# xin-fight/Research-and-Implementation-of-Image-Dehazing-Algorithm-Based-on-Vision-Transformer

Hardware: AMD Instinct MI355X
Metric: train patches/sec (128x128, embed_dim=32) (higher is better)
Workload: dtype f32; 1 GPU; Uformer_ProbSparse train step E=32 ps=128 per-GPU bs=32 fp32 Charbonnier+CR(VGG19, seeded-random weights) + AdamW (BASELINE configs[1]); global_batch=32, parallelism=dp1, arithmetic=fp32 storage/accumulate; products 6xbf16 MFMA, dropped <= 2^-24, split_terms=6

## Files before the change

### include/dehaze_hip.h

```cpp
#ifndef DEHAZE_HIP_H
#define DEHAZE_HIP_H

#include <stdint.h>

#ifdef __cplusplus
extern "C" {
#endif

#define DHZ_OK 0
#define DHZ_EINVAL (-22)
#define DHZ_ELAUNCH (-5)

#define DHZ_F32 0
#define DHZ_BF16 1

#define DHZ_NTOK 64
#define DHZ_NTOP 25

int dhz_abi_version(void);
const char* dhz_last_error(void);
const char* dhz_build_id(void);
int dhz_set_reserved_cus(int k);
int dhz_get_reserved_cus(void);
int dhz_grid_cus(void);
// ... 161 lines not shown
int dhz_linear_wgrad(const float* dy, int ldy, const float* x, int ldx, int T, int N, int K,
                     float* dw, float* db, void* stream);
int dhz_linear_wgrad_rs(const float* dy, int ldy, const float* x, int ldx, int T, int N, int K, float* dw, float* db,
                        const float* row_scale, int rows_per_scale, void* stream);
int dhz_linear_wgrad_multi(const float* dy, int ldy, const float* x, int ldx, int T, int nmat, int nper, int K,
                           float* const* dw, float* const* db, void* stream);

int dhz_winograd_prepack(const float* weight, float* upack, int Kout, int Cin, int transposed_rot, void* stream);
int dhz_winograd_conv3x3(const float* x, const float* upack, const float* bias, int relu, const float* out_mask,
                         const float* out_addend, float* y, int B, int H, int W, int C, int K, void* stream);
int dhz_winograd43_prepack(const float* weight, float* upack, int Kout, int Cin, int transposed_rot, void* stream);
int dhz_winograd43_conv3x3(const float* x, const float* upack, const float* bias, int relu, const float* out_mask,
                           const float* out_addend, float* y, int B, int H, int W, int C, int K, void* stream);
int dhz_winograd43_conv3x3_pool(const float* x, const float* upack, const float* bias, float* ypool, float* scratch, int B, int H, int W,
                                int C, int K, void* stream);
int dhz_maxpool2x2_blocked_fwd(const float* x, float* y, int N, int H, int W, void* stream);
int dhz_maxpool2x2_blocked_bwd(const float* gy, const float* act, float* gx, int N, int H, int W, void* stream);
int dhz_layout_blocked8(const float* src, float* dst, int B, int C, int HW, int to_blocked, const float* bias, int relu,
                        void* stream);

int dhz_winograd_conv3x3_act(const float* x, const float* upack, const float* bias, int backward, const float* out_mask,
                             const float* out_addend, float* y, int B, int H, int W, int C, int K, void* stream);

int dhz_tokens_to_blocked8(const float* tok, int ld, const float* leaky_mask, float* blk, int B, int HW, int C, void* stream);
int dhz_blocked8_to_tokens(const float* blk, const float* addend, int ld_add, float* tok, int ld, int B, int HW, int C, void* stream);

size_t dhz_conv3x3_wgrad_workspace_bytes(int B, int H, int W, int Cin, int Kout);
int dhz_conv3x3_wgrad_parts(int B, int H, int W, int Cin, int Kout);
int dhz_conv3x3_wgrad(const float* x, const float* dy, float* dw, float* db, float* ws, size_t ws_bytes, int B, int H, int W, int Cin,
                      int Kout, void* stream);
// ... 120 lines not shown
```

### research-and-implementation-of-image-dehazing-algorithm-based-on-vision-transformer_amd/csrc/common.h

```cpp
#pragma once
#include <hip/hip_runtime.h>
#include <stdint.h>
#include <stdio.h>
#include "dehaze_hip.h"

typedef float f32x4 __attribute__((ext_vector_type(4)));
typedef float f32x16 __attribute__((ext_vector_type(16)));

struct bf16s { uint16_t v; };
__device__ __forceinline__ float bf16_to_f32(uint16_t h) { return __uint_as_float((uint32_t)h << 16); }
__device__ __forceinline__ uint16_t f32_to_bf16(float f) {
    const __bf16 b = (__bf16)f;
    return __builtin_bit_cast(uint16_t, b);
}
__device__ __forceinline__ float4 ld4(const float* p) { return *reinterpret_cast<const float4*>(p); }
#ifndef DHZ_ST4_NT
#define DHZ_ST4_NT 0
#endif
__device__ __forceinline__ void st4(float* p, float4 v) {
    if (DHZ_ST4_NT) __builtin_nontemporal_store(f32x4{v.x, v.y, v.z, v.w}, reinterpret_cast<f32x4*>(p));
    else *reinterpret_cast<float4*>(p) = v;
}
__device__ __forceinline__ float4 ld4(const bf16s* p) {
    const uint2 r = *reinterpret_cast<const uint2*>(p);
// ... 23 lines not shown
bool dhz_det();
int dhz_part_cus();
constexpr int DHZ_DET_MAXSEG = 8;
struct DetSegs {
    int n;
    long off[DHZ_DET_MAXSEG], len[DHZ_DET_MAXSEG];
    float* dst[DHZ_DET_MAXSEG];
};
float* dhz_det_ws(const char* who, long items, long slot);
int dhz_det_reduce(const char* who, const float* ws, int items, long slot, const DetSegs& segs, hipStream_t s);
template <bool DET>
__device__ __forceinline__ void dhz_accum(float* p, float v) {
    if constexpr (DET) *p = v;
    else atomicAdd(p, v);
}

#define DHZ_REQUIRE(cond, ...)            \
    do {                                  \
        if (!(cond)) {                    \
            dhz_set_error(__VA_ARGS__);   \
            return DHZ_EINVAL;            \
        }                                 \
    } while (0)

#define DHZ_CHECK_LAUNCH(name)                                                   \
    do {                                                                         \
        hipError_t e_ = hipGetLastError();                                       \
        if (e_ != hipSuccess) {                                                  \
            dhz_set_error("%s: launch failed: %s", name, hipGetErrorString(e_)); \
            return DHZ_ELAUNCH;                                                  \
// ... 119 lines not shown
```

### research-and-implementation-of-image-dehazing-algorithm-based-on-vision-transformer_amd/csrc/winograd43_conv.hip

```cpp
#include <stdlib.h>
#include <type_traits>
#include "common.h"

#ifndef W43_ABL
#define W43_ABL 0
#endif

namespace {

typedef float f32x2 __attribute__((ext_vector_type(2)));
typedef __attribute__((address_space(3))) void lds_void;
typedef const __attribute__((address_space(1))) void glb_void;

constexpr int KB = 32;
constexpr int CC = 8;
constexpr int NXI = 36;
constexpr int UF = NXI * CC * KB;
constexpr int NUBUF = 2;
constexpr int URUNS = UF / 256;
static_assert(URUNS / 4 == 9, "the counted wait at the end of a group (vmcnt(9)) leaves exactly a wave's filter requests in flight");
constexpr int PLANE = 332;
constexpr int PCHUNKS = 2 * PLANE;
constexpr int PRUNS = (PCHUNKS + 63) / 64;
constexpr int PFLOATS = PRUNS * 256;
// ... 42 lines not shown
__global__ __launch_bounds__(256, 1) void winograd43_conv3x3_kernel(const float* __restrict__ x, const float* __restrict__ upack,
                                                                    const float* __restrict__ bias, int relu,
                                                                    const float* __restrict__ out_mask,
                                                                    const float* __restrict__ out_addend, float* __restrict__ y, int H,
                                                                    int W, int C, int K, int nblk, int xcd_group, int cb0, int ncb,
                                                                    int chain, float* __restrict__ ypool) {
    extern __shared__ __attribute__((aligned(16))) float smem[];
    const int t = threadIdx.x, lane = t & 63;
    const int w = __builtin_amdgcn_readfirstlane(t >> 6);
    const int i16 = lane & 15, g = lane >> 4;
    const int ty = i16 >> 2, tx = i16 & 3, hf = g >> 1, sub = g & 1;
    float* const us = smem;
    float* const pw = smem + NUBUF * UF + w * PFLOATS;
    float* const bias_s = smem + NUBUF * UF + 4 * PFLOATS;
    const int KBn = K / KB, CBn = C / CC;
    int lid = blockIdx.x;
    if (xcd_group) lid = (blockIdx.x & 7) * (gridDim.x >> 3) + (blockIdx.x >> 3);
    const int kb = lid % KBn;
    int blk = (lid / KBn) * 4 + w;
    const bool live = blk < nblk;
    if (!live) blk = nblk - 1;
    const int bx_n = W / 16, by_n = H / 16;
    const int bimg = blk / (bx_n * by_n);
    const int by = (blk / bx_n) % by_n, bx = blk % bx_n;
    const int oy0 = by * 16, ox0 = bx * 16;
    const size_t plane = (size_t)H * W * 8;

    {
        f32x4* z = reinterpret_cast<f32x4*>(pw);
#pragma unroll
        for (int i = 0; i < PFLOATS / 4 / 64; ++i) z[lane + 64 * i] = f32x4{0.f, 0.f, 0.f, 0.f};
    }
    if (FWD && t < KB) bias_s[t] = bias ? bias[kb * KB + t] : 0.f;

    int poff[PRUNS];
#pragma unroll
    for (int r = 0; r < PRUNS; ++r) {
        const int c = 64 * r + lane;
        const int ph = c / PLANE, rr = c - ph * PLANE;
        const int k4 = rr / 73;
        const int q = rr - 73 * k4;
        const int row = 4 * k4 + q / 18, px = q % 18;
        const int iy = oy0 - 1 + row, ix = ox0 - 1 + px;
        const bool ok = ph < 2 && q < 72 && row < 18 && iy >= 0 && iy < H && ix >= 0 && ix < W;
        poff[r] = ok ? (iy * W + ix) * 8 + ph * 4 : -1;
    }
    const char* const xbase = reinterpret_cast<const char*>(x + ((size_t)bimg * CBn + cb0) * plane);
    const char* const ubase = reinterpret_cast<const char*>(upack + ((size_t)kb * CBn + cb0) * UF);
    const unsigned lane16 = lane * 16;
    auto dma_patch_run = [&](int cb, int r) {
        if (W43_ABL & 2) return;
        if (poff[r] >= 0) dma16s(xbase + (size_t)cb * plane * 4, (unsigned)(poff[r] * 4), pw + 256 * r);
    };
    auto dma_u_run = [&](int cb, int r) {
        if (W43_ABL & 2) return;
        const int run = w + 4 * r;
        dma16s(ubase + ((size_t)cb * UF + 256 * run) * 4, lane16, us + (cb & 1) * UF + 256 * run);
    };

    const float* const pread0 = pw + (hf * PLANE + 73 * ty + 4 * tx) * 4 + 2 * sub;
    constexpr int NXA = 32;
    f32x4 acc[NXA][2], accv[NXI - NXA][2];
// ... 236 lines not shown
        (void)hipFuncSetAttribute(reinterpret_cast<const void*>(&winograd43_conv3x3_kernel<F>),                        \
                                  hipFuncAttributeMaxDynamicSharedMemorySize, (int)W43_SMEM);                          \
        for (int cb0 = 0; cb0 < CBn; cb0 += CHAIN_GROUPS) {                                                            \
            const int ncb = CBn - cb0 < CHAIN_GROUPS ? CBn - cb0 : CHAIN_GROUPS;                                       \
            const int chain = (cb0 > 0 ? 1 : 0) | (cb0 + ncb < CBn ? 2 : 0);                                           \
            hipLaunchKernelGGL((winograd43_conv3x3_kernel<F>), dim3(grid), dim3(256), W43_SMEM, s, x, upack, bias,     \
                               relu, out_mask, out_addend, y, H, W, C, K, nblk, xcd_group, cb0, ncb, chain, ypool);    \
        }                                                                                                              \
    } while (0)
    if (fwd) GO(true); else GO(false);
#undef GO
    DHZ_CHECK_LAUNCH(who);
    return DHZ_OK;
}

extern "C" int dhz_winograd43_conv3x3(const float* x, const float* upack, const float* bias, int relu, const float* out_mask,
                                      const float* out_addend, float* y, int B, int H, int W, int C, int K, void* stream) {
    DHZ_REQUIRE(y, "dhz_winograd43_conv3x3: null pointer");
    return winograd43_launch("dhz_winograd43_conv3x3", x, upack, bias, relu, out_mask, out_addend, y, nullptr, B, H, W, C, K, stream);
}

extern "C" int dhz_winograd43_conv3x3_pool(const float* x, const float* upack, const float* bias, float* ypool, float* scratch, int B, int H,
                                           int W, int C, int K, void* stream) {
    DHZ_REQUIRE(ypool, "dhz_winograd43_conv3x3_pool: null pointer");
    return winograd43_launch("dhz_winograd43_conv3x3_pool", x, upack, bias, 1, nullptr, nullptr, scratch, ypool, B, H, W, C, K, stream);
}
```

### research-and-implementation-of-image-dehazing-algorithm-based-on-vision-transformer_amd/csrc/winograd_conv.hip

```cpp
#include <stdlib.h>
#include <type_traits>
#include "common.h"

#ifndef WINO_ABL
#define WINO_ABL 0
#endif

namespace {

typedef float f32x2 __attribute__((ext_vector_type(2)));

constexpr int KB = 32;
constexpr int CC = 8;
constexpr int RS = 48;
constexpr int PPL = 320;
constexpr int UF = 16 * CC * KB;
constexpr int VW = 16 * 4 * 32;
constexpr int WAVE_LDS = VW + 4 * PPL;
constexpr int YS = 68;
constexpr int NP4 = 4;
constexpr int NUBUF = 3;
constexpr size_t WINO_SMEM = (size_t)(NUBUF * UF + 8 * WAVE_LDS + KB) * sizeof(float);

__device__ __forceinline__ void wave_sync() {
    __builtin_amdgcn_fence(__ATOMIC_RELEASE, "wavefront");
    __builtin_amdgcn_wave_barrier();
    __builtin_amdgcn_fence(__ATOMIC_ACQUIRE, "wavefront");
}

constexpr float LEAKY_SLOPE = 0.01f;
template <bool FWD, bool Q8, bool LEAKY = false>
__global__ __launch_bounds__(512) void winograd_conv3x3_kernel(const float* __restrict__ x,
                                                           const float* __restrict__ upack,
                                                           const float* __restrict__ bias, int relu,
                                                           const float* __restrict__ out_mask,
                                                           const float* __restrict__ out_addend,
                                                           float* __restrict__ y, int H, int W, int C, int K, int nblk, int xcd_group,
                                                           int nimg) {
    extern __shared__ __attribute__((aligned(16))) float smem[];
    const int t = threadIdx.x, lane = t & 63, w = t >> 6, half = w >> 2, wl = w & 3;
    const int i16 = lane & 15, g = lane >> 4;
    float* us = smem;
    float* vw = smem + NUBUF * UF + w * WAVE_LDS;
    float* pw = vw + VW;
    const int KBn = K / KB, CBn = C / CC;
    int lid = blockIdx.x;
    if (xcd_group) lid = (blockIdx.x & 7) * (gridDim.x >> 3) + (blockIdx.x >> 3);
    const int kb = lid % KBn;
    int blk = (lid / KBn) * 2 + half;
    const bool live = blk < nblk;
    if (!live) blk = nblk - 1;
    const int bx_n = Q8 ? 1 : W / 16, by_n = Q8 ? 1 : H / 16;
    const int bimg = Q8 ? 0 : blk / (bx_n * by_n);
    const int by = (blk / bx_n) % by_n, bx = blk % bx_n;
    const int wy0 = by * 16 + 4 * wl, ox0 = bx * 16;
    const size_t plane = (size_t)H * W * 8;
    const int pbar = half ? 5 : 1;

    f32x4 acc[16][2];
#pragma unroll
    for (int xi = 0; xi < 16; ++xi) { acc[xi][0] = f32x4{0.f, 0.f, 0.f, 0.f}; acc[xi][1] = f32x4{0.f, 0.f, 0.f, 0.f}; }

// ... 9 lines not shown
        const bool in = e < 6 * 18 * 2 && iy >= 0 && iy < (Q8 ? 16 : H) && ix >= 0 && ix < (Q8 ? 16 : W);
        if (Q8) {
            const int img = min(4 * blk + 2 * (iy >> 3) + (ix >> 3), nimg - 1);
            poff[i] = in ? (unsigned)(img * (C / CC) * 512 + ((iy & 7) * 8 + (ix & 7)) * 8 + hf * 4) : 0u;
        } else
            poff[i] = in ? (unsigned)((iy * W + ix) * 8 + hf * 4) : 0u;
        pdst[i] = (2 * hf) * PPL + (in ? py * RS + px * 2 : 6 * RS + (lane & 15) * 2);
    }
    {
        float4* z = reinterpret_cast<float4*>(pw);
#pragma unroll
        for (int i = 0; i < 4 * PPL / 4 / 64; ++i) z[lane + 64 * i] = make_float4(0.f, 0.f, 0.f, 0.f);
    }
    float4 rp[NP4];
    float4 ru0, ru1;
    const float* xbase = x + (size_t)bimg * CBn * plane;
    const float4* ubase = reinterpret_cast<const float4*>(upack + (size_t)kb * CBn * UF) + t;
    auto gload_patch = [&](int cb) {
        const float* xp = xbase + (size_t)cb * plane;
#pragma unroll
        for (int i = 0; i < NP4; ++i) rp[i] = *reinterpret_cast<const float4*>(xp + poff[i]);
    };
    auto gload_u = [&](int cb) {
        const float4* up = ubase + (size_t)cb * (UF / 4);
        ru0 = up[0]; ru1 = up[512];
    };
    auto write_patch_slot = [&](int i) {
        const float4 val = rp[i];
        float* dst = pw + pdst[i];
        *reinterpret_cast<float2*>(dst) = make_float2(val.x, val.y);
        *reinterpret_cast<float2*>(dst + PPL) = make_float2(val.z, val.w);
    };
// ... 37 lines not shown
    };
    auto write_v = [&]() {
#pragma unroll
        for (int xi = 0; xi < 16; xi += 2) write_v2(xi);
    };

    float* bias_s = smem + NUBUF * UF + 8 * WAVE_LDS;
    if (FWD && t < KB) bias_s[t] = bias ? bias[kb * KB + t] : 0.f;

    gload_patch(0);
    gload_u(0);
    wave_sync();
#pragma unroll
    for (int i = 0; i < NP4; ++i) write_patch_slot(i);
    write_u(0);
    { const int c1 = CBn > 1 ? 1 : 0; gload_patch(c1); gload_u(c1); }
    wave_sync();
#pragma unroll
    for (int a = 0; a < 4; ++a) read_row(a);
#pragma unroll
    for (int b = 0; b < 4; ++b) col_transform(b);
#pragma unroll
    for (int a = 0; a < 4; ++a) row_transform(a);
    write_v();
    __syncthreads();

    const float* ufrag = us + (g * 16 + i16) * 4;
    const float* vfrag = vw + g * 32 + i16 * 2;
    auto group = [&](int cb, auto with_next) {
        constexpr bool WITH_NEXT = decltype(with_next)::value;
        const float* up = ufrag + (cb % NUBUF) * UF;
        const int nbuf = (cb + 1) % NUBUF;
        const int cb2 = cb + 2 < CBn ? cb + 2 : CBn - 1;
        auto slot = [&](int sidx) {
            if (!WITH_NEXT) return;
            if ((WINO_ABL & 1) && sidx >= 13 && sidx <= 21) return;
            if ((WINO_ABL & 2) && (sidx == 1 || sidx == 6)) { if (sidx == 6) wave_sync(); return; }
            if ((WINO_ABL & 8) && (sidx == 0 || (sidx >= 2 && sidx <= 5) || (sidx >= 8 && sidx <= 11) || sidx >= 22)) return;
            switch (sidx) {
                case 0: write_u(nbuf); break;
                case 1: gload_u(cb2); break;
                case 2: write_patch_slot(0); break;
                case 3: write_patch_slot(1); break;
                case 4: write_patch_slot(2); break;
                case 5: write_patch_slot(3); break;
                case 6: wave_sync(); gload_patch(cb2); break;
                case 8: read_row(0); break;
                case 9: read_row(1); break;
// ... 50 lines not shown
            __builtin_amdgcn_sched_barrier(0);
            slot(4 * j + 2);
            __builtin_amdgcn_sched_barrier(0);
            if (!(WINO_ABL & 4)) {
            acc[xi + 1][0] = mfma16(a1.y, b1.y, acc[xi + 1][0]);
            acc[xi + 1][1] = mfma16(a1.w, b1.y, acc[xi + 1][1]); } else { acc[xi + 1][1][0] += a1.y + b1.y + a1.z + a1.w; }
            __builtin_amdgcn_sched_barrier(0);
            slot(4 * j + 3);
            __builtin_amdgcn_sched_barrier(0);
            a0 = a0n; a1 = a1n; b0 = b0n; b1 = b1n;
        }
        wave_sync();
        if (WITH_NEXT && !(WINO_ABL & 8)) { write_v2(12); write_v2(14); }
        wave_sync();
    };
    for (int cb = 0; cb + 1 < CBn; ++cb) group(cb, std::true_type{});
    group(CBn - 1, std::false_type{});

    float* ys = vw;
    {
        const int ty = i16 >> 3, tx = i16 & 7;
        const float lo = relu ? 0.f : -__builtin_inff();
#pragma unroll
        for (int tr = 0; tr < 2; ++tr)
#pragma unroll
            for (int r = 0; r < 4; ++r) {
                const int k = 16 * tr + 4 * g + r;
                float m[16];
#pragma unroll
                for (int xi = 0; xi < 16; ++xi) m[xi] = acc[xi][tr][r];
                float t0[4], t1[4];
#pragma unroll
// ... 4 lines not shown
                const float bv = FWD ? bias_s[k] : 0.f;
                float y00 = t0[0] + t0[1] + t0[2] + bv, y01 = t0[1] - t0[2] - t0[3] + bv;
                float y10 = t1[0] + t1[1] + t1[2] + bv, y11 = t1[1] - t1[2] - t1[3] + bv;
                if (FWD && LEAKY) {
                    y00 = y00 > 0.f ? y00 : LEAKY_SLOPE * y00; y01 = y01 > 0.f ? y01 : LEAKY_SLOPE * y01;
                    y10 = y10 > 0.f ? y10 : LEAKY_SLOPE * y10; y11 = y11 > 0.f ? y11 : LEAKY_SLOPE * y11;
                } else if (FWD) { y00 = fmaxf(y00, lo); y01 = fmaxf(y01, lo); y10 = fmaxf(y10, lo); y11 = fmaxf(y11, lo); }
                float* o = ys + k * YS + (2 * ty) * 16 + 2 * tx;
                *reinterpret_cast<float2*>(o) = make_float2(y00, y01);
                *reinterpret_cast<float2*>(o + 16) = make_float2(y10, y11);
            }
    }
    wave_sync();
    if (live) {
        const int KG = K / 8;
#pragma unroll
        for (int i = 0; i < 8; ++i) {
            const int e = lane + 64 * i;
            const int hf = e & 1, px = (e >> 1) & 15, py = (e >> 5) & 3, kg = e >> 7;
            const float* s0 = ys + (kg * 8 + hf * 4) * YS + py * 16 + px;
            float4 v4 = make_float4(s0[0], s0[YS], s0[2 * YS], s0[3 * YS]);
            size_t o;
            if (Q8) {
                const int vy = wy0 + py, img = 4 * blk + 2 * (vy >> 3) + (px >> 3);
                if (img >= nimg) continue;
                o = ((((size_t)img * KG + kb * 4 + kg) * 8 + (vy & 7)) * 8 + (px & 7)) * 8 + hf * 4;
            } else
                o = (((size_t)bimg * KG + kb * 4 + kg) * H + wy0 + py) * W * 8 + (size_t)(ox0 + px) * 8 + hf * 4;
            if (!FWD || LEAKY) {
                if (out_addend) {
// ... 3 lines not shown
                if (LEAKY && !FWD && out_mask) {
                    const float4 m = *reinterpret_cast<const float4*>(out_mask + o);
                    v4.x = m.x > 0.f ? v4.x : LEAKY_SLOPE * v4.x; v4.y = m.y > 0.f ? v4.y : LEAKY_SLOPE * v4.y;
                    v4.z = m.z > 0.f ? v4.z : LEAKY_SLOPE * v4.z; v4.w = m.w > 0.f ? v4.w : LEAKY_SLOPE * v4.w;
                } else if (!FWD && out_mask) {
                    const float4 m = *reinterpret_cast<const float4*>(out_mask + o);
                    v4.x = m.x > 0.f ? v4.x : 0.f; v4.y = m.y > 0.f ? v4.y : 0.f;
                    v4.z = m.z > 0.f ? v4.z : 0.f; v4.w = m.w > 0.f ? v4.w : 0.f;
                }
            }
            *reinterpret_cast<float4*>(y + o) = v4;
        }
    }
}

__global__ void winograd_prepack_kernel(const float* __restrict__ wgt, float* __restrict__ upack, int Kout, int Cin,
                                        int transposed_rot) {
    const int e = blockIdx.x * blockDim.x + threadIdx.x;
    if (e >= Kout * Cin) return;
    const int k = e / Cin, c = e % Cin;
    float gk[3][3];
#pragma unroll
    for (int i = 0; i < 3; ++i)
#pragma unroll
        for (int j = 0; j < 3; ++j)
            gk[i][j] = transposed_rot ? wgt[((size_t)c * Kout + k) * 9 + (2 - i) * 3 + (2 - j)]
                                      : wgt[((size_t)k * Cin + c) * 9 + i * 3 + j];
    float tg[4][3];
#pragma unroll
    for (int j = 0; j < 3; ++j) {
// ... 121 lines not shown
    gx[o] = ra; gx[o + 2] = rb; gx[o + 2 * W] = rc; gx[o + 2 * W + 2] = rd;
}

}

extern "C" int dhz_winograd_prepack(const float* weight, float* upack, int Kout, int Cin, int transposed_rot,
                                    void* stream) {
    DHZ_REQUIRE(weight && upack && Kout % KB == 0 && Cin % CC == 0, "dhz_winograd_prepack: Kout=%d Cin=%d", Kout, Cin);
    const int n = Kout * Cin;
    hipLaunchKernelGGL(winograd_prepack_kernel, dim3((n + 255) / 256), dim3(256), 0, (hipStream_t)stream, weight, upack,
                       Kout, Cin, transposed_rot);
    DHZ_CHECK_LAUNCH("dhz_winograd_prepack");
    return DHZ_OK;
}

extern "C" int dhz_winograd_conv3x3(const float* x, const float* upack, const float* bias, int relu, const float* out_mask,
                                    const float* out_addend, float* y, int B, int H, int W, int C, int K, void* stream) {
    DHZ_REQUIRE(x && upack && y, "dhz_winograd_conv3x3: null pointer");
    const bool q8 = H == 8 && W == 8;
    DHZ_REQUIRE(B > 0 && ((H % 16 == 0 && W % 16 == 0) || q8) && C % CC == 0 && K % KB == 0,
                "dhz_winograd_conv3x3: unsupported shape B=%d H=%d W=%d C=%d K=%d", B, H, W, C, K);
    const bool fwd = !(out_mask || out_addend);
    DHZ_REQUIRE(fwd || !(bias || relu), "dhz_winograd_conv3x3: bias/relu and out_mask/out_addend are exclusive");
    const int nblk = q8 ? (B + 3) / 4 : B * (H / 16) * (W / 16);
    const int grid = ((nblk + 1) / 2) * (K / KB);
    hipStream_t s = (hipStream_t)stream;
#ifdef DHZ_DIAG
    static const int xcd_env = getenv("DHZ_WINO_XCD") ? atoi(getenv("DHZ_WINO_XCD")) : -1;
#else
    constexpr int xcd_env = -1;
#endif
    const int xcd_group = (grid % 8 == 0) && (xcd_env >= 0 ? xcd_env : 1);
#define GO(F, Q)                                                                                                   \
    do {                                                                                                           \
        (void)hipFuncSetAttribute(reinterpret_cast<const void*>(&winograd_conv3x3_kernel<F, Q>),                   \
                                  hipFuncAttributeMaxDynamicSharedMemorySize, (int)WINO_SMEM);                     \
        hipLaunchKernelGGL((winograd_conv3x3_kernel<F, Q>), dim3(grid), dim3(512), WINO_SMEM, s, x, upack, bias, relu, \
                           out_mask, out_addend, y, H, W, C, K, nblk, xcd_group, B);                               \
    } while (0)
    if (q8) { if (fwd) GO(true, true); else GO(false, true); }
    else { if (fwd) GO(true, false); else GO(false, false); }
#undef GO
    DHZ_CHECK_LAUNCH("dhz_winograd_conv3x3");
    return DHZ_OK;
}

extern "C" int dhz_winograd_conv3x3_act(const float* x, const float* upack, const float* bias, int backward, const float* out_mask,
                                        const float* out_addend, float* y, int B, int H, int W, int C, int K, void* stream) {
    DHZ_REQUIRE(x && upack && y, "dhz_winograd_conv3x3_act: null pointer");
    const bool q8 = H == 8 && W == 8;
    DHZ_REQUIRE(B > 0 && ((H % 16 == 0 && W % 16 == 0 && H > 0 && W > 0) || q8) && C > 0 && K > 0 && C % CC == 0 && K % KB == 0,
                "dhz_winograd_conv3x3_act: unsupported shape B=%d H=%d W=%d C=%d K=%d", B, H, W, C, K);
    DHZ_REQUIRE(backward ? (bias == nullptr && out_mask != nullptr) : out_mask == nullptr,
                "dhz_winograd_conv3x3_act: forward takes bias / out_addend, backward out_mask / out_addend");
    const int nblk = q8 ? (B + 3) / 4 : B * (H / 16) * (W / 16);
    const int grid = ((nblk + 1) / 2) * (K / KB);
    hipStream_t s = (hipStream_t)stream;
    const int xcd_group = grid % 8 == 0;
#define GO(F, Q)                                                                                                         \
    do {                                                                                                                 \
        (void)hipFuncSetAttribute(reinterpret_cast<const void*>(&winograd_conv3x3_kernel<F, Q, true>),                   \
                                  hipFuncAttributeMaxDynamicSharedMemorySize, (int)WINO_SMEM);                           \
        hipLaunchKernelGGL((winograd_conv3x3_kernel<F, Q, true>), dim3(grid), dim3(512), WINO_SMEM, s, x, upack, bias, 0, \
                           out_mask, out_addend, y, H, W, C, K, nblk, xcd_group, B);                                     \
    } while (0)
    if (q8) { if (!backward) GO(true, true); else GO(false, true); }
    else { if (!backward) GO(true, false); else GO(false, false); }
#undef GO
    DHZ_CHECK_LAUNCH("dhz_winograd_conv3x3_act");
    return DHZ_OK;
}

extern "C" int dhz_layout_blocked8(const float* src, float* dst, int B, int C, int HW, int to_blocked, const float* bias,
                                   int relu, void* stream) {
    DHZ_REQUIRE(src && dst && C % 8 == 0 && B > 0 && HW > 0, "dhz_layout_blocked8: bad arguments");
    DHZ_REQUIRE(to_blocked || !(bias || relu), "dhz_layout_blocked8: bias / relu only towards the blocked layout");
    const size_t n = (size_t)B * C * HW;
    if (HW % 4 == 0) {
        const size_t total = n / 32;
// ... 29 lines not shown
```

### research-and-implementation-of-image-dehazing-algorithm-based-on-vision-transformer_amd/dehaze_hip/_lib.py

```python
import ctypes
import os

_HERE = os.path.dirname(os.path.abspath(__file__))
LIB_PATH = os.environ.get("DHZ_LIB_PATH") or os.path.join(_HERE, "libdehaze_hip.so")

c_f = ctypes.c_void_p
c_p = ctypes.c_void_p
c_i = ctypes.c_int
c_l = ctypes.c_int64
c_fl = ctypes.c_float

SIGNATURES = {
    "dhz_abi_version": [],
    "dhz_last_error": [],
    "dhz_build_id": [],
    "dhz_set_reserved_cus": [ctypes.c_int],
    "dhz_gelu_fwd_dt": [ctypes.c_void_p, ctypes.c_void_p, ctypes.c_int64, ctypes.c_int, ctypes.c_void_p],
    "dhz_gelu_bwd_dt": [ctypes.c_void_p, ctypes.c_void_p, ctypes.c_void_p, ctypes.c_int64, ctypes.c_void_p, ctypes.c_int64, ctypes.c_int, ctypes.c_void_p],
    "dhz_get_reserved_cus": [],
    "dhz_set_deterministic": [ctypes.c_int],
    "dhz_get_deterministic": [],
    "dhz_set_det_workspace": [ctypes.c_void_p, ctypes.c_size_t],
    "dhz_grid_cus": [],
    "dhz_ps_attn_fwd": [c_f, c_f, c_f, c_i, c_p, c_f, c_f, c_f, c_i, c_p, c_i, c_i, c_i, c_i, c_p],
# ... 21 lines not shown
    "dhz_thin_conv3x3_fwd": [c_f, c_f, c_f, c_f, c_i, c_i, c_i, c_i, c_p],
    "dhz_thin_conv3x3_dgrad": [c_f, c_f, c_f, c_i, c_i, c_i, c_i, c_p],
    "dhz_conv3x3_in3_blocked": [c_f, c_f, c_f, c_f, c_i, c_i, c_i, c_i, c_i, c_p],
    "dhz_thin_conv3x3_dgrad_blocked": [c_f, c_f, c_f, c_i, c_i, c_i, c_i, c_p],
    "dhz_thin_conv3x3_wgrad": [c_f, c_f, c_f, c_f, c_i, c_i, c_i, c_i, c_p],
    "dhz_l1_pair_fwd": [c_f, c_f, c_f, c_f, c_l, c_p],
    "dhz_l1_pair_bwd": [c_f, c_f, c_f, c_f, c_f, c_l, c_p],
    "dhz_contrast_combine_fwd": [c_f, c_f, c_f, c_i, c_i, c_f, c_f, c_p],
    "dhz_contrast_combine_bwd": [c_f, c_f, c_i, c_i, c_f, c_f, c_f, c_f, c_p],
    "dhz_crop_augment_pair": [c_f, c_f, c_f, c_f, c_f, c_i, c_i, c_i, c_i, c_p],
    "dhz_winograd_prepack": [c_f, c_f, c_i, c_i, c_i, c_p],
    "dhz_winograd_conv3x3": [c_f, c_f, c_f, c_i, c_f, c_f, c_f, c_i, c_i, c_i, c_i, c_i, c_p],
    "dhz_winograd43_prepack": [c_f, c_f, c_i, c_i, c_i, c_p],
    "dhz_winograd43_conv3x3": [c_f, c_f, c_f, c_i, c_f, c_f, c_f, c_i, c_i, c_i, c_i, c_i, c_p],
    "dhz_winograd43_conv3x3_pool": [c_f, c_f, c_f, c_f, c_f, c_i, c_i, c_i, c_i, c_i, c_p],
    "dhz_maxpool2x2_blocked_fwd": [c_f, c_f, c_i, c_i, c_i, c_p],
    "dhz_maxpool2x2_blocked_bwd": [c_f, c_f, c_f, c_i, c_i, c_i, c_p],
    "dhz_layout_blocked8": [c_f, c_f, c_i, c_i, c_i, c_i, c_f, c_i, c_p],
    "dhz_leff_fused_fwd": [c_f] * 16 + [c_i, c_i, c_i, c_i, c_p],
    "dhz_leff_fused_fwd6": [c_f] * 15 + [c_i, c_i, c_i, c_i, c_p],
    "dhz_leff_prepack6": [c_f, c_f, c_p, c_i, c_p],
    "dhz_linear_fwd": [c_f, c_i, c_f, c_f, c_f, c_i, c_i, c_i, c_i, c_p],
    "dhz_linear_dgrad": [c_f, c_i, c_f, c_f, c_i, c_i, c_i, c_i, c_p],
    "dhz_input_proj_fwd": [c_f, c_f, c_f, c_f, c_i, c_i, c_i, c_i, c_fl, c_p],
    "dhz_input_proj_bwd": [c_f, c_f, c_f, c_f, c_f, c_i, c_i, c_i, c_i, c_fl, c_p],
    "dhz_conv4s2_fwd": [c_f, c_f, c_f, c_f, c_i, c_i, c_i, c_i, c_i, c_p],
    "dhz_conv4s2_dgrad": [c_f, c_f, c_f, c_i, c_i, c_i, c_i, c_i, c_p],
    "dhz_conv4s2_wgrad": [c_f, c_f, c_f, c_f, c_i, c_i, c_i, c_i, c_i, c_p],
    "dhz_input_proj_fwd_dt": [c_f, c_f, c_f, c_f, c_i, c_i, c_i, c_i, c_fl, c_i, c_p],
    "dhz_input_proj_bwd_dt": [c_f, c_f, c_f, c_f, c_f, c_i, c_i, c_i, c_i, c_fl, c_i, c_p],
# ... 127 lines not shown
```

### research-and-implementation-of-image-dehazing-algorithm-based-on-vision-transformer_amd/dehaze_hip/vgg.py

```python
import os

import torch
import torch.nn.functional as F
from torch.autograd import Function

from . import _lib
from . import ops
from .ops import _p, _stream

CONVS = ((3, 64), (64, 64), (64, 128), (128, 128), (128, 256), (256, 256), (256, 256), (256, 256), (256, 512),
         (512, 512), (512, 512), (512, 512), (512, 512))
POOL_AFTER = (1, 3, 7, 11)
TAPS = (0, 2, 4, 8, 12)


def wino_supported(H, W):
    return (H % 16 == 0 and W % 16 == 0) or (H == 8 and W == 8)


def to_blocked(x, bias=None, relu=False):
    B, C, H, W = x.shape
    out = torch.empty((B, C // 8, H, W, 8), device=x.device, dtype=torch.float32)
    _lib.call("dhz_layout_blocked8", _p(x.contiguous()), _p(out), B, C, H * W, 1, _p(bias), int(relu), _stream())
    return out
# ... 27 lines not shown

F43_ON = os.environ.get("DHZ_WINO_F43", "1") != "0"


F43_DIFF = os.environ.get("DHZ_WINO_F43_DIFF", "1") != "0"
POOL_FUSED = os.environ.get("DHZ_WINO_POOL", "1") != "0"


def use_f43(B, H, W, Cin, Kout):
    if not F43_ON or H % 16 or W % 16 or H < 16 or W < 16 or Cin % 16 or Kout % 32:
        return False
    wgs = (B * (H // 16) * (W // 16) + 3) // 4 * (Kout // 32)
    cus = _lib.load().dhz_grid_cus() + _lib.load().dhz_get_reserved_cus()
    rounds = (wgs + cus - 1) // cus
    return wgs >= 0.92 * rounds * cus


class VggEngine:
    def __init__(self, convs):
        self.convs = convs
        self._packed = {}
        self._packed43 = {}

    def packed(self, i, device):
        key = (i, str(device), self.convs[i].weight.data_ptr(), self.convs[i].weight._version)
        hit = self._packed.get(i)
        if hit is None or hit[0] != key:
            w = self.convs[i].weight.detach().contiguous()
            K, C = w.shape[0], w.shape[1]
            uf = torch.empty(16 * K * C, device=device, dtype=torch.float32)
# ... 10 lines not shown
        if hit is None or hit[0] != key:
            w = self.convs[i].weight.detach().contiguous()
            K, C = w.shape[0], w.shape[1]
            uf = torch.empty(36 * K * C, device=device, dtype=torch.float32)
            ub = torch.empty(36 * K * C, device=device, dtype=torch.float32)
            _lib.call("dhz_winograd43_prepack", _p(w), _p(uf), K, C, 0, _stream())
            _lib.call("dhz_winograd43_prepack", _p(w), _p(ub), C, K, 1, _stream())
            hit = (key, uf, ub)
            self._packed43[i] = hit
        return hit[1], hit[2]

    def conv(self, i, xb, allow43=True, pool=False):
        B, CG, H, W, _ = xb.shape
        C, K = CONVS[i]
        f43 = allow43 and use_f43(B, H, W, C, K)
        uf, _ = self.packed43(i, xb.device) if f43 else self.packed(i, xb.device)
        if pool and f43:
            yp = torch.empty((B, K // 8, H // 2, W // 2, 8), device=xb.device, dtype=torch.float32)
            scratch = torch.empty((B, K // 8, H, W, 8), device=xb.device, dtype=torch.float32) if C > 256 else None
            ev = ops._timed("dhz_winograd_conv3x3")
            _lib.call("dhz_winograd43_conv3x3_pool", _p(xb), _p(uf), _p(self.convs[i].bias), _p(yp), _p(scratch) if scratch is not None else None,
                      B, H, W, C, K, _stream())
            _timing_end(ev, B, H, W, C, K, f43)
            return yp
        yb = torch.empty((B, K // 8, H, W, 8), device=xb.device, dtype=torch.float32)
        ev = ops._timed("dhz_winograd_conv3x3")
        _lib.call("dhz_winograd43_conv3x3" if f43 else "dhz_winograd_conv3x3", _p(xb), _p(uf), _p(self.convs[i].bias), 1, None, None,
                  _p(yb), B, H, W, C, K, _stream())
        _timing_end(ev, B, H, W, C, K, f43)
        return pool_fwd(yb) if pool else yb

    def conv_dgrad(self, i, gb, below_act=None, addend=None):
        B, KG, H, W, _ = gb.shape
        C, K = CONVS[i]
        f43 = use_f43(B, H, W, K, C)
        _, ub = self.packed43(i, gb.device) if f43 else self.packed(i, gb.device)
        dxb = torch.empty((B, C // 8, H, W, 8), device=gb.device, dtype=torch.float32)
        ev = ops._timed("dhz_winograd_conv3x3")
        _lib.call("dhz_winograd43_conv3x3" if f43 else "dhz_winograd_conv3x3", _p(gb), _p(ub), None, 0,
                  _p(below_act) if below_act is not None else None,
                  _p(addend.contiguous()) if addend is not None else None, _p(dxb), B, H, W, K, C, _stream())
        _timing_end(ev, B, H, W, K, C, f43)
        return dxb

    def forward_taps(self, x, save=None):
        c0 = self.convs[0]
        xc = x.contiguous()
        cur = torch.empty((xc.shape[0], 8, xc.shape[2], xc.shape[3], 8), device=x.device, dtype=torch.float32)
        _lib.call("dhz_conv3x3_in3_blocked", _p(xc), _p(c0.weight.contiguous()), _p(c0.bias), _p(cur), xc.shape[0], xc.shape[2],
                  xc.shape[3], 64, 1, _stream())
        acts = {0: cur}
        taps = [cur]
        x12 = None
        for i in range(1, 13):
            if i == 12 and not wino_supported(cur.shape[2], cur.shape[3]):
                c12 = self.convs[12]
                ops.warn_library_fallback("VGG19 conv5_1", tuple(cur.shape))
# ... 302 lines not shown
```

Baseline: 1004 patches/s.

## Split Winograd VGG convs over input-channel slices with a reduction epilogue

Adds split-K style slicing of the Winograd F(2,3) and F(4,3) conv kernels over input-channel groups. Each slice writes raw partial sums to a workspace, and a separate epilogue kernel sums them and applies bias/ReLU or mask/addend. Slicing is chosen only when the normal grid underfills the CUs, so deep low-resolution VGG layers get more workgroups. The cost is extra workspace traffic, one more kernel launch per conv, and a different summation order.

```diff
diff --git a/include/dehaze_hip.h b/include/dehaze_hip.h
--- a/include/dehaze_hip.h
+++ b/include/dehaze_hip.h
@@ -199,6 +199,13 @@
                            const float* out_addend, float* y, int B, int H, int W, int C, int K, void* stream);
 int dhz_winograd43_conv3x3_pool(const float* x, const float* upack, const float* bias, float* ypool, float* scratch, int B, int H, int W,
                                 int C, int K, void* stream);
+int dhz_winograd_conv3x3_slices(const float* x, const float* upack, const float* bias, int relu, const float* out_mask,
+                                const float* out_addend, float* y, float* workspace, int slices, int B, int H, int W, int C, int K,
+                                void* stream);
+int dhz_winograd43_conv3x3_slices(const float* x, const float* upack, const float* bias, int relu, const float* out_mask,
+                                  const float* out_addend, float* y, float* workspace, int slices, int B, int H, int W, int C, int K,
+                                  void* stream);
+int dhz_winograd_slices(int B, int H, int W, int C, int K);
 int dhz_maxpool2x2_blocked_fwd(const float* x, float* y, int N, int H, int W, void* stream);
 int dhz_maxpool2x2_blocked_bwd(const float* gy, const float* act, float* gx, int N, int H, int W, void* stream);
 int dhz_layout_blocked8(const float* src, float* dst, int B, int C, int HW, int to_blocked, const float* bias, int relu,
diff --git a/research-and-implementation-of-image-dehazing-algorithm-based-on-vision-transformer_amd/csrc/common.h b/research-and-implementation-of-image-dehazing-algorithm-based-on-vision-transformer_amd/csrc/common.h
--- a/research-and-implementation-of-image-dehazing-algorithm-based-on-vision-transformer_amd/csrc/common.h
+++ b/research-and-implementation-of-image-dehazing-algorithm-based-on-vision-transformer_amd/csrc/common.h
@@ -61,6 +61,9 @@
     if constexpr (DET) *p = v;
     else atomicAdd(p, v);
 }
+
+int dhz_wino_slices_epilogue(const char* who, const float* ws, int slices, const float* bias, int relu, const float* out_mask,
+                             const float* out_addend, float* y, int B, int H, int W, int K, hipStream_t s);
 
 #define DHZ_REQUIRE(cond, ...)            \
     do {                                  \
diff --git a/research-and-implementation-of-image-dehazing-algorithm-based-on-vision-transformer_amd/csrc/winograd43_conv.hip b/research-and-implementation-of-image-dehazing-algorithm-based-on-vision-transformer_amd/csrc/winograd43_conv.hip
--- a/research-and-implementation-of-image-dehazing-algorithm-based-on-vision-transformer_amd/csrc/winograd43_conv.hip
+++ b/research-and-implementation-of-image-dehazing-algorithm-based-on-vision-transformer_amd/csrc/winograd43_conv.hip
@@ -80,6 +80,8 @@
     float* const pw = smem + NUBUF * UF + w * PFLOATS;
     float* const bias_s = smem + NUBUF * UF + 4 * PFLOATS;
     const int KBn = K / KB, CBn = C / CC;
+    const int sl = blockIdx.y;
+    cb0 += sl * ncb;
     int lid = blockIdx.x;
     if (xcd_group) lid = (blockIdx.x & 7) * (gridDim.x >> 3) + (blockIdx.x >> 3);
     const int kb = lid % KBn;
@@ -87,7 +89,8 @@
     const bool live = blk < nblk;
     if (!live) blk = nblk - 1;
     const int bx_n = W / 16, by_n = H / 16;
-    const int bimg = blk / (bx_n * by_n);
+    const int bimg_in = blk / (bx_n * by_n);
+    const int bimg = bimg_in + sl * (nblk / (bx_n * by_n));
     const int by = (blk / bx_n) % by_n, bx = blk % bx_n;
     const int oy0 = by * 16, ox0 = bx * 16;
     const size_t plane = (size_t)H * W * 8;
@@ -111,7 +114,7 @@
         const bool ok = ph < 2 && q < 72 && row < 18 && iy >= 0 && iy < H && ix >= 0 && ix < W;
         poff[r] = ok ? (iy * W + ix) * 8 + ph * 4 : -1;
     }
-    const char* const xbase = reinterpret_cast<const char*>(x + ((size_t)bimg * CBn + cb0) * plane);
+    const char* const xbase = reinterpret_cast<const char*>(x + ((size_t)bimg_in * CBn + cb0) * plane);
     const char* const ubase = reinterpret_cast<const char*>(upack + ((size_t)kb * CBn + cb0) * UF);
     const unsigned lane16 = lane * 16;
     auto dma_patch_run = [&](int cb, int r) {
@@ -378,6 +381,31 @@
     return DHZ_OK;
 }
 
+extern "C" int dhz_winograd43_conv3x3_slices(const float* x, const float* upack, const float* bias, int relu, const float* out_mask,
+                                             const float* out_addend, float* y, float* workspace, int slices, int B, int H, int W, int C,
+                                             int K, void* stream) {
+    const char* who = "dhz_winograd43_conv3x3_slices";
+    DHZ_REQUIRE(x && upack && y && workspace, "%s: null pointer", who);
+    DHZ_REQUIRE(B > 0 && H % 16 == 0 && W % 16 == 0 && H >= 16 && W >= 16 && C > 0 && K > 0 && C % 16 == 0 && K % KB == 0,
+                "%s: unsupported shape B=%d H=%d W=%d C=%d K=%d", who, B, H, W, C, K);
+    const bool fwd = !(out_mask || out_addend);
+    DHZ_REQUIRE(fwd || !(bias || relu), "%s: bias/relu and out_mask/out_addend are exclusive", who);
+    DHZ_REQUIRE((long long)H * W * 8 * (C / 8) < (1ll << 31), "%s: image too large", who);
+    const int CBn = C / CC;
+    DHZ_REQUIRE(slices >= 2 && slices <= 64 && CBn % slices == 0 && CBn / slices <= CHAIN_GROUPS,
+                "%s: slices=%d of %d channel groups (equal ranges of at most %d)", who, slices, CBn, CHAIN_GROUPS);
+    const long long nblk = (long long)B * (H / 16) * (W / 16);
+    const long long grid1 = ((nblk + 3) / 4) * (K / KB);
+    DHZ_REQUIRE(grid1 * slices < (1ll << 31) && nblk * slices < (1ll << 31) / 4, "%s: grid too large", who);
+    const int xcd_group = (grid1 % 8 == 0) ? 1 : 0;
+    (void)hipFuncSetAttribute(reinterpret_cast<const void*>(&winograd43_conv3x3_kernel<false>), hipFuncAttributeMaxDynamicSharedMemorySize,
+                              (int)W43_SMEM);
+    hipLaunchKernelGGL((winograd43_conv3x3_kernel<false>), dim3((unsigned)grid1, (unsigned)slices), dim3(256), W43_SMEM, (hipStream_t)stream,
+                       x, upack, nullptr, 0, nullptr, nullptr, workspace, H, W, C, K, (int)nblk, xcd_group, 0, CBn / slices, 2, nullptr);
+    DHZ_CHECK_LAUNCH(who);
+    return dhz_wino_slices_epilogue(who, workspace, slices, bias, relu, out_mask, out_addend, y, B, H, W, K, (hipStream_t)stream);
+}
+
 extern "C" int dhz_winograd43_conv3x3(const float* x, const float* upack, const float* bias, int relu, const float* out_mask,
                                       const float* out_addend, float* y, int B, int H, int W, int C, int K, void* stream) {
     DHZ_REQUIRE(y, "dhz_winograd43_conv3x3: null pointer");
diff --git a/research-and-implementation-of-image-dehazing-algorithm-based-on-vision-transformer_amd/csrc/winograd_conv.hip b/research-and-implementation-of-image-dehazing-algorithm-based-on-vision-transformer_amd/csrc/winograd_conv.hip
--- a/research-and-implementation-of-image-dehazing-algorithm-based-on-vision-transformer_amd/csrc/winograd_conv.hip
+++ b/research-and-implementation-of-image-dehazing-algorithm-based-on-vision-transformer_amd/csrc/winograd_conv.hip
@@ -29,14 +29,14 @@
 }
 
 constexpr float LEAKY_SLOPE = 0.01f;
-template <bool FWD, bool Q8, bool LEAKY = false>
+template <bool FWD, bool Q8, bool LEAKY = false, bool RAW = false>
 __global__ __launch_bounds__(512) void winograd_conv3x3_kernel(const float* __restrict__ x,
                                                            const float* __restrict__ upack,
                                                            const float* __restrict__ bias, int relu,
                                                            const float* __restrict__ out_mask,
                                                            const float* __restrict__ out_addend,
                                                            float* __restrict__ y, int H, int W, int C, int K, int nblk, int xcd_group,
-                                                           int nimg) {
+                                                           int nimg, int slices) {
     extern __shared__ __attribute__((aligned(16))) float smem[];
     const int t = threadIdx.x, lane = t & 63, w = t >> 6, half = w >> 2, wl = w & 3;
     const int i16 = lane & 15, g = lane >> 4;
@@ -44,8 +44,13 @@
     float* vw = smem + NUBUF * UF + w * WAVE_LDS;
     float* pw = vw + VW;
     const int KBn = K / KB, CBn = C / CC;
-    int lid = blockIdx.x;
-    if (xcd_group) lid = (blockIdx.x & 7) * (gridDim.x >> 3) + (blockIdx.x >> 3);
+    static_assert(!RAW || (!FWD && !LEAKY), "the raw store is the backward instance without mask and addend");
+    const int grid1 = RAW ? (int)gridDim.x / slices : (int)gridDim.x;
+    const int sl = RAW ? (int)blockIdx.x / grid1 : 0;
+    int lid = RAW ? (int)blockIdx.x - sl * grid1 : (int)blockIdx.x;
+    if (xcd_group) lid = (lid & 7) * (grid1 >> 3) + (lid >> 3);
+    const int cbs = RAW ? sl * CBn / slices : 0;
+    const int NG = RAW ? (sl + 1) * CBn / slices - cbs : CBn;
     const int kb = lid % KBn;
     int blk = (lid / KBn) * 2 + half;
     const bool live = blk < nblk;
@@ -85,8 +90,8 @@
     }
     float4 rp[NP4];
     float4 ru0, ru1;
-    const float* xbase = x + (size_t)bimg * CBn * plane;
-    const float4* ubase = reinterpret_cast<const float4*>(upack + (size_t)kb * CBn * UF) + t;
+    const float* xbase = x + ((size_t)bimg * CBn + cbs) * plane;
+    const float4* ubase = reinterpret_cast<const float4*>(upack + ((size_t)kb * CBn + cbs) * UF) + t;
     auto gload_patch = [&](int cb) {
         const float* xp = xbase + (size_t)cb * plane;
 #pragma unroll
@@ -154,7 +159,7 @@
 #pragma unroll
     for (int i = 0; i < NP4; ++i) write_patch_slot(i);
     write_u(0);
-    { const int c1 = CBn > 1 ? 1 : 0; gload_patch(c1); gload_u(c1); }
+    { const int c1 = NG > 1 ? 1 : 0; gload_patch(c1); gload_u(c1); }
     wave_sync();
 #pragma unroll
     for (int a = 0; a < 4; ++a) read_row(a);
@@ -171,7 +176,7 @@
         constexpr bool WITH_NEXT = decltype(with_next)::value;
         const float* up = ufrag + (cb % NUBUF) * UF;
         const int nbuf = (cb + 1) % NUBUF;
-        const int cb2 = cb + 2 < CBn ? cb + 2 : CBn - 1;
+        const int cb2 = cb + 2 < NG ? cb + 2 : NG - 1;
         auto slot = [&](int sidx) {
             if (!WITH_NEXT) return;
             if ((WINO_ABL & 1) && sidx >= 13 && sidx <= 21) return;
@@ -252,8 +257,8 @@
         if (WITH_NEXT && !(WINO_ABL & 8)) { write_v2(12); write_v2(14); }
         wave_sync();
     };
-    for (int cb = 0; cb + 1 < CBn; ++cb) group(cb, std::true_type{});
-    group(CBn - 1, std::false_type{});
+    for (int cb = 0; cb + 1 < NG; ++cb) group(cb, std::true_type{});
+    group(NG - 1, std::false_type{});
 
     float* ys = vw;
     {
@@ -288,6 +293,7 @@
     wave_sync();
     if (live) {
         const int KG = K / 8;
+        if (RAW) y += (size_t)sl * nimg * K * H * W;
 #pragma unroll
         for (int i = 0; i < 8; ++i) {
             const int e = lane + 64 * i;
@@ -321,6 +327,40 @@
     }
 }
 
+template <bool FWD>
+__global__ __launch_bounds__(256) void winograd_slices_epilogue_kernel(const float4* __restrict__ ws, size_t n4, int slices,
+                                                                       const float* __restrict__ bias, int relu,
+                                                                       const float4* __restrict__ out_mask,
+                                                                       const float4* __restrict__ out_addend, float4* __restrict__ y,
+                                                                       int HW, int KG) {
+    const size_t e = (size_t)blockIdx.x * 256 + threadIdx.x;
+    if (e >= n4) return;
+    float4 r = make_float4(0.f, 0.f, 0.f, 0.f);
+    if (slices > 1) r = ws[e];
+    for (int s = 1; s + 1 < slices; ++s) {
+        const float4 p = ws[(size_t)s * n4 + e];
+        r.x += p.x; r.y += p.y; r.z += p.z; r.w += p.w;
+    }
+    float4 v = ws[(size_t)(slices - 1) * n4 + e];
+    if (FWD) {
+        float4 b = make_float4(0.f, 0.f, 0.f, 0.f);
+        if (bias) b = *reinterpret_cast<const float4*>(bias + ((e >> 1) / HW % KG) * 8 + (e & 1) * 4);
+        v.x += b.x; v.y += b.y; v.z += b.z; v.w += b.w;
+    }
+    if (slices > 1) { v.x += r.x; v.y += r.y; v.z += r.z; v.w += r.w; }
+    if (FWD) {
+        const float lo = relu ? 0.f : -__builtin_inff();
+        v.x = fmaxf(v.x, lo); v.y = fmaxf(v.y, lo); v.z = fmaxf(v.z, lo); v.w = fmaxf(v.w, lo);
+    } else {
+        if (out_addend) { const float4 ad = out_addend[e]; v.x += ad.x; v.y += ad.y; v.z += ad.z; v.w += ad.w; }
+        if (out_mask) {
+            const float4 m = out_mask[e];
+            v.x = m.x > 0.f ? v.x : 0.f; v.y = m.y > 0.f ? v.y : 0.f; v.z = m.z > 0.f ? v.z : 0.f; v.w = m.w > 0.f ? v.w : 0.f;
+        }
+    }
+    y[e] = v;
+}
+
 __global__ void winograd_prepack_kernel(const float* __restrict__ wgt, float* __restrict__ upack, int Kout, int Cin,
                                         int transposed_rot) {
     const int e = blockIdx.x * blockDim.x + threadIdx.x;
@@ -472,14 +512,33 @@
     return DHZ_OK;
 }
 
-extern "C" int dhz_winograd_conv3x3(const float* x, const float* upack, const float* bias, int relu, const float* out_mask,
-                                    const float* out_addend, float* y, int B, int H, int W, int C, int K, void* stream) {
-    DHZ_REQUIRE(x && upack && y, "dhz_winograd_conv3x3: null pointer");
+int dhz_wino_slices_epilogue(const char* who, const float* ws, int slices, const float* bias, int relu, const float* out_mask,
+                             const float* out_addend, float* y, int B, int H, int W, int K, hipStream_t s) {
+    const size_t n4 = (size_t)B * K * H * W / 4;
+    const dim3 grid((unsigned)((n4 + 255) / 256));
+    if (!(out_mask || out_addend))
+        hipLaunchKernelGGL(winograd_slices_epilogue_kernel<true>, grid, dim3(256), 0, s, reinterpret_cast<const float4*>(ws), n4, slices,
+                           bias, relu, nullptr, nullptr, reinterpret_cast<float4*>(y), H * W, K / 8);
+    else
+        hipLaunchKernelGGL(winograd_slices_epilogue_kernel<false>, grid, dim3(256), 0, s, reinterpret_cast<const float4*>(ws), n4, slices,
+                           nullptr, 0, reinterpret_cast<const float4*>(out_mask), reinterpret_cast<const float4*>(out_addend),
+                           reinterpret_cast<float4*>(y), H * W, K / 8);
+    DHZ_CHECK_LAUNCH(who);
+    return DHZ_OK;
+}
+
+constexpr int SLICE_MIN_GROUPS = 16;
+
+static int winograd_launch(const char* who, const float* x, const float* upack, const float* bias, int relu, const float* out_mask,
+                           const float* out_addend, float* y, float* ws, int slices, int B, int H, int W, int C, int K, void* stream) {
+    DHZ_REQUIRE(x && upack && y, "%s: null pointer", who);
     const bool q8 = H == 8 && W == 8;
     DHZ_REQUIRE(B > 0 && ((H % 16 == 0 && W % 16 == 0) || q8) && C % CC == 0 && K % KB == 0,
-                "dhz_winograd_conv3x3: unsupported shape B=%d H=%d W=%d C=%d K=%d", B, H, W, C, K);
+                "%s: unsupported shape B=%d H=%d W=%d C=%d K=%d", who, B, H, W, C, K);
     const bool fwd = !(out_mask || out_addend);
-    DHZ_REQUIRE(fwd || !(bias || relu), "dhz_winograd_conv3x3: bias/relu and out_mask/out_addend are exclusive");
+    DHZ_REQUIRE(fwd || !(bias || relu), "%s: bias/relu and out_mask/out_addend are exclusive", who);
+    DHZ_REQUIRE(slices >= 1 && slices <= C / CC && (slices == 1 || ws), "%s: slices=%d of %d channel groups, workspace %s", who, slices,
+                C / CC, ws ? "given" : "null");
     const int nblk = q8 ? (B + 3) / 4 : B * (H / 16) * (W / 16);
     const int grid = ((nblk + 1) / 2) * (K / KB);
     hipStream_t s = (hipStream_t)stream;
@@ -494,13 +553,50 @@
         (void)hipFuncSetAttribute(reinterpret_cast<const void*>(&winograd_conv3x3_kernel<F, Q>),                   \
                                   hipFuncAttributeMaxDynamicSharedMemorySize, (int)WINO_SMEM);                     \
         hipLaunchKernelGGL((winograd_conv3x3_kernel<F, Q>), dim3(grid), dim3(512), WINO_SMEM, s, x, upack, bias, relu, \
-                           out_mask, out_addend, y, H, W, C, K, nblk, xcd_group, B);                               \
+                           out_mask, out_addend, y, H, W, C, K, nblk, xcd_group, B, 1);                            \
     } while (0)
+#define GO_RAW(Q)                                                                                                  \
+    do {                                                                                                           \
+        (void)hipFuncSetAttribute(reinterpret_cast<const void*>(&winograd_conv3x3_kernel<false, Q, false, true>),  \
+                                  hipFuncAttributeMaxDynamicSharedMemorySize, (int)WINO_SMEM);                     \
+        hipLaunchKernelGGL((winograd_conv3x3_kernel<false, Q, false, true>), dim3(grid * slices), dim3(512), WINO_SMEM, s, x, upack, \
+                           nullptr, 0, nullptr, nullptr, ws, H, W, C, K, nblk, xcd_group, B, slices);              \
+    } while (0)
+    if (slices > 1) {
+        DHZ_REQUIRE((long long)grid * slices < (1ll << 31), "%s: grid too large", who);
+        if (q8) GO_RAW(true); else GO_RAW(false);
+        DHZ_CHECK_LAUNCH(who);
+        return dhz_wino_slices_epilogue(who, ws, slices, bias, relu, out_mask, out_addend, y, B, H, W, K, s);
+    }
     if (q8) { if (fwd) GO(true, true); else GO(false, true); }
     else { if (fwd) GO(true, false); else GO(false, false); }
 #undef GO
-    DHZ_CHECK_LAUNCH("dhz_winograd_conv3x3");
+#undef GO_RAW
+    DHZ_CHECK_LAUNCH(who);
     return DHZ_OK;
+}
+
+extern "C" int dhz_winograd_conv3x3(const float* x, const float* upack, const float* bias, int relu, const float* out_mask,
+                                    const float* out_addend, float* y, int B, int H, int W, int C, int K, void* stream) {
+    return winograd_launch("dhz_winograd_conv3x3", x, upack, bias, relu, out_mask, out_addend, y, nullptr, 1, B, H, W, C, K, stream);
+}
+
+extern "C" int dhz_winograd_conv3x3_slices(const float* x, const float* upack, const float* bias, int relu, const float* out_mask,
+                                           const float* out_addend, float* y, float* workspace, int slices, int B, int H, int W, int C,
+                                           int K, void* stream) {
+    return winograd_launch("dhz_winograd_conv3x3_slices", x, upack, bias, relu, out_mask, out_addend, y, workspace, slices, B, H, W, C, K,
+                           stream);
+}
+
+extern "C" int dhz_winograd_slices(int B, int H, int W, int C, int K) {
+    const bool q8 = H == 8 && W == 8;
+    if (B <= 0 || !((H % 16 == 0 && W % 16 == 0 && H > 0 && W > 0) || q8) || C <= 0 || K <= 0 || C % CC || K % KB) return 1;
+    const long long nblk = q8 ? (B + 3) / 4 : (long long)B * (H / 16) * (W / 16);
+    const long long grid = ((nblk + 1) / 2) * (K / KB);
+    const int cus = dhz_grid_cus() + dhz_get_reserved_cus();
+    for (int S = 4; S > 1; S >>= 1)
+        if (S * grid <= cus && (C / CC) / S >= SLICE_MIN_GROUPS) return S;
+    return 1;
 }
 
 extern "C" int dhz_winograd_conv3x3_act(const float* x, const float* upack, const float* bias, int backward, const float* out_mask,
@@ -520,7 +616,7 @@
         (void)hipFuncSetAttribute(reinterpret_cast<const void*>(&winograd_conv3x3_kernel<F, Q, true>),                   \
                                   hipFuncAttributeMaxDynamicSharedMemorySize, (int)WINO_SMEM);                           \
         hipLaunchKernelGGL((winograd_conv3x3_kernel<F, Q, true>), dim3(grid), dim3(512), WINO_SMEM, s, x, upack, bias, 0, \
-                           out_mask, out_addend, y, H, W, C, K, nblk, xcd_group, B);                                     \
+                           out_mask, out_addend, y, H, W, C, K, nblk, xcd_group, B, 1);                                  \
     } while (0)
     if (q8) { if (!backward) GO(true, true); else GO(false, true); }
     else { if (!backward) GO(true, false); else GO(false, false); }
diff --git a/research-and-implementation-of-image-dehazing-algorithm-based-on-vision-transformer_amd/dehaze_hip/_lib.py b/research-and-implementation-of-image-dehazing-algorithm-based-on-vision-transformer_amd/dehaze_hip/_lib.py
--- a/research-and-implementation-of-image-dehazing-algorithm-based-on-vision-transformer_amd/dehaze_hip/_lib.py
+++ b/research-and-implementation-of-image-dehazing-algorithm-based-on-vision-transformer_amd/dehaze_hip/_lib.py
@@ -59,6 +59,9 @@
     "dhz_winograd43_prepack": [c_f, c_f, c_i, c_i, c_i, c_p],
     "dhz_winograd43_conv3x3": [c_f, c_f, c_f, c_i, c_f, c_f, c_f, c_i, c_i, c_i, c_i, c_i, c_p],
     "dhz_winograd43_conv3x3_pool": [c_f, c_f, c_f, c_f, c_f, c_i, c_i, c_i, c_i, c_i, c_p],
+    "dhz_winograd_conv3x3_slices": [c_f, c_f, c_f, c_i, c_f, c_f, c_f, c_f, c_i, c_i, c_i, c_i, c_i, c_i, c_p],
+    "dhz_winograd43_conv3x3_slices": [c_f, c_f, c_f, c_i, c_f, c_f, c_f, c_f, c_i, c_i, c_i, c_i, c_i, c_i, c_p],
+    "dhz_winograd_slices": [c_i, c_i, c_i, c_i, c_i],
     "dhz_maxpool2x2_blocked_fwd": [c_f, c_f, c_i, c_i, c_i, c_p],
     "dhz_maxpool2x2_blocked_bwd": [c_f, c_f, c_f, c_i, c_i, c_i, c_p],
     "dhz_layout_blocked8": [c_f, c_f, c_i, c_i, c_i, c_i, c_f, c_i, c_p],
diff --git a/research-and-implementation-of-image-dehazing-algorithm-based-on-vision-transformer_amd/dehaze_hip/vgg.py b/research-and-implementation-of-image-dehazing-algorithm-based-on-vision-transformer_amd/dehaze_hip/vgg.py
--- a/research-and-implementation-of-image-dehazing-algorithm-based-on-vision-transformer_amd/dehaze_hip/vgg.py
+++ b/research-and-implementation-of-image-dehazing-algorithm-based-on-vision-transformer_amd/dehaze_hip/vgg.py
@@ -65,6 +65,46 @@
     cus = _lib.load().dhz_grid_cus() + _lib.load().dhz_get_reserved_cus()
     rounds = (wgs + cus - 1) // cus
     return wgs >= 0.92 * rounds * cus
+
+
+SLICES_ON = os.environ.get("DHZ_WINO_SLICES", "1") != "0"
+
+
+def _physical_cus():
+    return _lib.load().dhz_grid_cus() + _lib.load().dhz_get_reserved_cus()
+
+
+def f43_slices_rule(B, H, W, Cin, Kout, cus):
+    if H % 16 or W % 16 or H < 16 or W < 16 or Cin % 16 or Kout % 32:
+        return 0
+    wgs = (B * (H // 16) * (W // 16) + 3) // 4 * (Kout // 32)
+    rounds = (wgs + cus - 1) // cus
+    if wgs >= 0.92 * rounds * cus:
+        return 0
+    CBn = Cin // 8
+    for S in (2, 4):
+        if CBn % S == 0 and SLICE_MIN_GROUPS <= CBn // S <= 32 and 0.92 * cus <= S * wgs <= cus:
+            return S
+    return 0
+
+
+def use_f43_slices(B, H, W, Cin, Kout):
+    return f43_slices_rule(B, H, W, Cin, Kout, _physical_cus()) if (F43_ON and SLICES_ON) else 0
+
+
+SLICE_MIN_GROUPS = 16
+
+
+def wino_slices_rule(B, H, W, C, K, cus):
+    q8 = H == 8 and W == 8
+    if B <= 0 or not ((H % 16 == 0 and W % 16 == 0 and H > 0) or q8) or C % 8 or K % 32:
+        return 1
+    nblk = (B + 3) // 4 if q8 else B * (H // 16) * (W // 16)
+    grid = (nblk + 1) // 2 * (K // 32)
+    for S in (4, 2):
+        if S * grid <= cus and (C // 8) // S >= SLICE_MIN_GROUPS:
+            return S
+    return 1
 
 
 class VggEngine:
@@ -105,7 +145,9 @@
         B, CG, H, W, _ = xb.shape
         C, K = CONVS[i]
         f43 = allow43 and use_f43(B, H, W, C, K)
-        uf, _ = self.packed43(i, xb.device) if f43 else self.packed(i, xb.device)
+        s43 = use_f43_slices(B, H, W, C, K) if (allow43 and not f43) else 0
+        s22 = _lib.load().dhz_winograd_slices(B, H, W, C, K) if (SLICES_ON and not f43 and not s43) else 1
+        uf, _ = self.packed43(i, xb.device) if (f43 or s43) else self.packed(i, xb.device)
         if pool and f43:
             yp = torch.empty((B, K // 8, H // 2, W // 2, 8), device=xb.device, dtype=torch.float32)
             scratch = torch.empty((B, K // 8, H, W, 8), device=xb.device, dtype=torch.float32) if C > 256 else None
@@ -116,22 +158,35 @@
             return yp
         yb = torch.empty((B, K // 8, H, W, 8), device=xb.device, dtype=torch.float32)
         ev = ops._timed("dhz_winograd_conv3x3")
-        _lib.call("dhz_winograd43_conv3x3" if f43 else "dhz_winograd_conv3x3", _p(xb), _p(uf), _p(self.convs[i].bias), 1, None, None,
-                  _p(yb), B, H, W, C, K, _stream())
-        _timing_end(ev, B, H, W, C, K, f43)
+        if s43 or s22 > 1:
+            ws = torch.empty((s43 or s22, B, K // 8, H, W, 8), device=xb.device, dtype=torch.float32)
+            _lib.call("dhz_winograd43_conv3x3_slices" if s43 else "dhz_winograd_conv3x3_slices", _p(xb), _p(uf), _p(self.convs[i].bias), 1,
+                      None, None, _p(yb), _p(ws), s43 or s22, B, H, W, C, K, _stream())
+        else:
+            _lib.call("dhz_winograd43_conv3x3" if f43 else "dhz_winograd_conv3x3", _p(xb), _p(uf), _p(self.convs[i].bias), 1, None, None,
+                      _p(yb), B, H, W, C, K, _stream())
+        _timing_end(ev, B, H, W, C, K, f43 or bool(s43))
         return pool_fwd(yb) if pool else yb
 
     def conv_dgrad(self, i, gb, below_act=None, addend=None):
         B, KG, H, W, _ = gb.shape
         C, K = CONVS[i]
         f43 = use_f43(B, H, W, K, C)
-        _, ub = self.packed43(i, gb.device) if f43 else self.packed(i, gb.device)
+        s43 = 0 if f43 else use_f43_slices(B, H, W, K, C)
+        s22 = _lib.load().dhz_winograd_slices(B, H, W, K, C) if (SLICES_ON and not f43 and not s43) else 1
+        _, ub = self.packed43(i, gb.device) if (f43 or s43) else self.packed(i, gb.device)
         dxb = torch.empty((B, C // 8, H, W, 8), device=gb.device, dtype=torch.float32)
+        mask = _p(below_act) if below_act is not None else None
+        add = addend.contiguous() if addend is not None else None
         ev = ops._timed("dhz_winograd_conv3x3")
-        _lib.call("dhz_winograd43_conv3x3" if f43 else "dhz_winograd_conv3x3", _p(gb), _p(ub), None, 0,
-                  _p(below_act) if below_act is not None else None,
-                  _p(addend.contiguous()) if addend is not None else None, _p(dxb), B, H, W, K, C, _stream())
-        _timing_end(ev, B, H, W, K, C, f43)
+        if s43 or s22 > 1:
+            ws = torch.empty((s43 or s22, B, C // 8, H, W, 8), device=gb.device, dtype=torch.float32)
+            _lib.call("dhz_winograd43_conv3x3_slices" if s43 else "dhz_winograd_conv3x3_slices", _p(gb), _p(ub), None, 0, mask,
+                      _p(add) if add is not None else None, _p(dxb), _p(ws), s43 or s22, B, H, W, K, C, _stream())
+        else:
+            _lib.call("dhz_winograd43_conv3x3" if f43 else "dhz_winograd_conv3x3", _p(gb), _p(ub), None, 0, mask,
+                      _p(add) if add is not None else None, _p(dxb), B, H, W, K, C, _stream())
+        _timing_end(ev, B, H, W, K, C, f43 or bool(s43))
         return dxb
 
     def forward_taps(self, x, save=None):
```

Result: faster. 1024 patches/s (median of 6 runs) (+2.1%).
